# IN2-ViAUn/Exploration-of-Potential

Hardware: AMD Instinct MI355X
Metric: training images/sec, YOLOX-l 24p 640x640 bf16 (higher is better)
Workload: dtype bf16; 1 GPU; YOLOX-l-24p (CSPDarknet53+PAFPN+24p head) train step, 640x640, batch 20/GPU, 10 GTs/img, SimOTA + 24-circle GIoU loss, SGD nesterov; global_batch=20, parallelism=dp1, hip_graph=forward and backward as two lanes of captured segments, loss, update

## Files before the change

exploration-of-potential_amd/csrc/elementwise.hip:

```cpp
#include <stdio.h>
#include <stdlib.h>
#include "common.h"

namespace {

constexpr int MAX_BLOCKS = 2048;

__device__ __forceinline__ void load8(const bf16* p, float (&v)[8]) {
    bf16x8 t = *reinterpret_cast<const bf16x8*>(p);
#pragma unroll
    for (int i = 0; i < 8; ++i) v[i] = (float)t[i];
}
__device__ __forceinline__ void store8(bf16* p, const float (&v)[8]) {
    bf16x8 t;
#pragma unroll
    for (int i = 0; i < 8; ++i) t[i] = (bf16)v[i];
    *reinterpret_cast<bf16x8*>(p) = t;
}

__device__ __forceinline__ long pinned_row(long m) {
    asm volatile("" : "+v"(m));
    return m;
}

// ... 481 lines not shown
            const int yy = py + dy;
            if (yy < 0 || yy >= H) continue;
            for (int dx = -6; dx <= 6; ++dx) {
                const int xx = px + dx;
                if (xx < 0 || xx >= W) continue;
                float v[8];
                load8(x + ((long)(n * H + yy) * W + xx) * ld_x + cg * 8, v);
                const uint8_t code = (uint8_t)(((dy + 8) << 4) | (dx + 8));
                const bool in9 = dy >= -4 && dy <= 4 && dx >= -4 && dx <= 4;
                const bool in5 = dy >= -2 && dy <= 2 && dx >= -2 && dx <= 2;
#pragma unroll
                for (int j = 0; j < 8; ++j) {
                    if (v[j] > m13[j] || v[j] != v[j]) { m13[j] = v[j]; i13[j] = code; }
                    if (in9 && (v[j] > m9[j] || v[j] != v[j])) { m9[j] = v[j]; i9[j] = code; }
                    if (in5 && (v[j] > m5[j] || v[j] != v[j])) { m5[j] = v[j]; i5[j] = code; }
                }
            }
        }
        store8(y5 + pix * ld_y + cg * 8, m5);
        store8(y9 + pix * ld_y + cg * 8, m9);
        store8(y13 + pix * ld_y + cg * 8, m13);
        uint8_t* ip = idx + pix * C + cg * 8;
#pragma unroll
        for (int j = 0; j < 8; ++j) { ip[j] = i5[j]; ip[plane + j] = i9[j]; ip[2 * plane + j] = i13[j]; }
    }
}

__global__ __launch_bounds__(256) void spp_row_kernel(const bf16* x, long ld_x, bf16* h, uint8_t* hx, int B, int H, int W, int C) {
    const int cgs = C >> 3;
    const long total = (long)B * H * W * cgs;
    const long plane = (long)B * H * W * C;
    for (long i = (long)blockIdx.x * 256 + threadIdx.x; i < total; i += (long)gridDim.x * 256) {
        const int cg = (int)(i % cgs);
        const long pix = i / cgs;
        const int px = (int)(pix % W);
        float m5[8], m9[8], m13[8];
        uint8_t i5[8], i9[8], i13[8];
#pragma unroll
        for (int j = 0; j < 8; ++j) { m5[j] = m9[j] = m13[j] = -INFINITY; i5[j] = i9[j] = i13[j] = 8; }
#pragma unroll
        for (int dx = -6; dx <= 6; ++dx) {
            const int xx = px + dx;
            if (xx < 0 || xx >= W) continue;
            float v[8];
            load8(x + (pix + dx) * ld_x + cg * 8, v);
            const uint8_t code = (uint8_t)(dx + 8);
            const bool in9 = dx >= -4 && dx <= 4, in5 = dx >= -2 && dx <= 2;
#pragma unroll
            for (int j = 0; j < 8; ++j) {
                if (v[j] > m13[j] || v[j] != v[j]) { m13[j] = v[j]; i13[j] = code; }
                if (in9 && (v[j] > m9[j] || v[j] != v[j])) { m9[j] = v[j]; i9[j] = code; }
                if (in5 && (v[j] > m5[j] || v[j] != v[j])) { m5[j] = v[j]; i5[j] = code; }
            }
        }
        bf16* hp = h + pix * C + cg * 8;
        store8(hp, m5); store8(hp + plane, m9); store8(hp + 2 * plane, m13);
        uint8_t* ip = hx + pix * C + cg * 8;
#pragma unroll
        for (int j = 0; j < 8; ++j) { ip[j] = i5[j]; ip[plane + j] = i9[j]; ip[2 * plane + j] = i13[j]; }
    }
}

__global__ __launch_bounds__(256) void spp_col_kernel(const bf16* h, const uint8_t* hx, bf16* y5, bf16* y9, bf16* y13, long ld_y,
                                                      uint8_t* idx, int B, int H, int W, int C) {
    const int cgs = C >> 3;
    const long total = (long)B * H * W * cgs;
    const long plane = (long)B * H * W * C;
    for (long i = (long)blockIdx.x * 256 + threadIdx.x; i < total; i += (long)gridDim.x * 256) {
        const int cg = (int)(i % cgs);
        const long pix = i / cgs;
        const int py = (int)((pix / W) % H);
        float m[3][8];
        uint8_t id[3][8];
#pragma unroll
        for (int w = 0; w < 3; ++w)
#pragma unroll
            for (int j = 0; j < 8; ++j) { m[w][j] = -INFINITY; id[w][j] = 0x88; }
#pragma unroll
        for (int dy = -6; dy <= 6; ++dy) {
            const int yy = py + dy;
            if (yy < 0 || yy >= H) continue;
            const long q = (pix + (long)dy * W) * C + cg * 8;
#pragma unroll
            for (int w = 0; w < 3; ++w) {
                const int r = 2 + 2 * w;
                if (dy < -r || dy > r) continue;
                float v[8];
                load8(h + w * plane + q, v);
                const uint2 cx = *reinterpret_cast<const uint2*>(hx + w * plane + q);
#pragma unroll
                for (int j = 0; j < 8; ++j) {
                    const unsigned c = ((j < 4 ? cx.x : cx.y) >> (8 * (j & 3))) & 0xFF;
                    if (v[j] > m[w][j] || v[j] != v[j]) { m[w][j] = v[j]; id[w][j] = (uint8_t)(((dy + 8) << 4) | c); }
                }
            }
        }
        store8(y5 + pix * ld_y + cg * 8, m[0]);
        store8(y9 + pix * ld_y + cg * 8, m[1]);
        store8(y13 + pix * ld_y + cg * 8, m[2]);
        uint8_t* ip = idx + pix * C + cg * 8;
#pragma unroll
        for (int j = 0; j < 8; ++j) { ip[j] = id[0][j]; ip[plane + j] = id[1][j]; ip[2 * plane + j] = id[2][j]; }
    }
}

__global__ __launch_bounds__(256) void spp_bwd_kernel(const bf16* dy5, const bf16* dy9, const bf16* dy13, long ld_dy,
                                                      const uint8_t* idx, bf16* dx, long ld_dx, int accumulate, int B,
                                                      int H, int W, int C) {
    const int cgs = C >> 3;
    const long total = (long)B * H * W * cgs;
    const long plane = (long)B * H * W * C;
    for (long i = (long)blockIdx.x * 256 + threadIdx.x; i < total; i += (long)gridDim.x * 256) {
        const int cg = (int)(i % cgs);
        const long pix = i / cgs;
        const int n = (int)(pix / (H * W));
        const int rem = (int)(pix - (long)n * H * W);
        const int py = rem / W, px = rem - py * W;
        float acc[8] = {0, 0, 0, 0, 0, 0, 0, 0};
        for (int dy = -6; dy <= 6; ++dy) {
            const int oy = py - dy;
            if (oy < 0 || oy >= H) continue;
            for (int dxo = -6; dxo <= 6; ++dxo) {
                const int ox = px - dxo;
                if (ox < 0 || ox >= W) continue;
                const long op = (long)(n * H + oy) * W + ox;
                const uint8_t code = (uint8_t)(((dy + 8) << 4) | (dxo + 8));
                const uint8_t* ip = idx + op * C + cg * 8;
                const unsigned rep = code * 0x01010101u;
                auto gather = [&](const bf16* g, const uint8_t* codes) {
                    uint2 c = *reinterpret_cast<const uint2*>(codes);
                    c.x ^= rep; c.y ^= rep;
                    float v[8];
                    load8(g + op * ld_dy + cg * 8, v);
#pragma unroll
                    for (int j = 0; j < 8; ++j)
                        if ((((j < 4 ? c.x : c.y) >> (8 * (j & 3))) & 0xFFu) == 0u) acc[j] += v[j];
                };
                gather(dy13, ip + 2 * plane);
                if (dy >= -4 && dy <= 4 && dxo >= -4 && dxo <= 4) gather(dy9, ip + plane);
                if (dy >= -2 && dy <= 2 && dxo >= -2 && dxo <= 2) gather(dy5, ip);
            }
        }
        bf16* d = dx + pix * ld_dx + cg * 8;
        if (accumulate) {
            float o[8];
            load8(d, o);
#pragma unroll
            for (int j = 0; j < 8; ++j) acc[j] += o[j];
        }
        store8(d, acc);
    }
}

__global__ __launch_bounds__(256) void spp_bwd_lds_kernel(const bf16* dy5, const bf16* dy9, const bf16* dy13, long ld_dy,
                                                          const uint8_t* idx, bf16* dx, long ld_dx, int accumulate, int B,
                                                          int H, int W, int C) {
    extern __shared__ __attribute__((aligned(16))) char spp_lds[];
    const int HW = H * W;
    bf16x8* gv = reinterpret_cast<bf16x8*>(spp_lds);
    uint2* cv = reinterpret_cast<uint2*>(spp_lds + (size_t)3 * HW * 16);
    float* gh = reinterpret_cast<float*>(spp_lds + (size_t)3 * HW * 24);
    uint2* ds = reinterpret_cast<uint2*>(spp_lds + (size_t)3 * HW * 24 + (size_t)HW * 32);
    const int cg = blockIdx.x, n = blockIdx.y;
    const long plane = (long)B * HW * C;
    const long base = (long)n * HW;
    for (int q = threadIdx.x; q < HW; q += 256) {
        const long op = base + q;
        gv[q] = *reinterpret_cast<const bf16x8*>(dy5 + op * ld_dy + cg * 8);
        gv[HW + q] = *reinterpret_cast<const bf16x8*>(dy9 + op * ld_dy + cg * 8);
        gv[2 * HW + q] = *reinterpret_cast<const bf16x8*>(dy13 + op * ld_dy + cg * 8);
        const uint8_t* ip = idx + op * C + cg * 8;
        cv[q] = *reinterpret_cast<const uint2*>(ip);
        cv[HW + q] = *reinterpret_cast<const uint2*>(ip + plane);
        cv[2 * HW + q] = *reinterpret_cast<const uint2*>(ip + 2 * plane);
    }
    __syncthreads();
    constexpr int NPASS = 4;
    float acc[NPASS][8];
#pragma unroll
    for (int t = 0; t < NPASS; ++t)
#pragma unroll
        for (int j = 0; j < 8; ++j) acc[t][j] = 0.f;
    for (int pool = 2; pool >= 0; --pool) {
        const int R = 2 * pool + 2;
        for (int q = threadIdx.x; q < HW; q += 256) {
            const int r = q / W, x = q - r * W;
            float s[8] = {0, 0, 0, 0, 0, 0, 0, 0};
            unsigned char sel[8];
#pragma unroll
            for (int j = 0; j < 8; ++j) sel[j] = 0xFF;
            for (int dy = -R; dy <= R; ++dy) {
                const int y = r - dy;
                if (y < 0 || y >= H) continue;
                const int o = y * W + x;
                const uint2 c = cv[pool * HW + o];
                const bf16x8 t = gv[pool * HW + o];
#pragma unroll
                for (int j = 0; j < 8; ++j) {
                    const unsigned byte = ((j < 4 ? c.x : c.y) >> (8 * (j & 3))) & 0xFFu;
                    if ((int)(byte >> 4) == dy + 8) { s[j] += (float)t[j]; sel[j] = (unsigned char)(byte & 15u); }
                }
            }
#pragma unroll
            for (int j = 0; j < 8; ++j) gh[q * 8 + j] = s[j];
            uint2 d;
            d.x = sel[0] | (sel[1] << 8) | (sel[2] << 16) | ((unsigned)sel[3] << 24);
            d.y = sel[4] | (sel[5] << 8) | (sel[6] << 16) | ((unsigned)sel[7] << 24);
            ds[q] = d;
        }
        __syncthreads();
#pragma unroll
        for (int t = 0; t < NPASS; ++t) {
            const int q = threadIdx.x + 256 * t;
            if (q < HW) {
                const int r = q / W, c = q - r * W;
                for (int dxo = -R; dxo <= R; ++dxo) {
                    const int x = c - dxo;
                    if (x < 0 || x >= W) continue;
                    const int o = r * W + x;
                    const uint2 d = ds[o];
#pragma unroll
                    for (int j = 0; j < 8; ++j) {
                        const unsigned byte = ((j < 4 ? d.x : d.y) >> (8 * (j & 3))) & 0xFFu;
                        if ((int)byte == dxo + 8) acc[t][j] += gh[o * 8 + j];
                    }
                }
            }
        }
        __syncthreads();
    }
#pragma unroll
    for (int t = 0; t < NPASS; ++t) {
        const int q = threadIdx.x + 256 * t;
        if (q < HW) {
            bf16* d = dx + (base + q) * ld_dx + cg * 8;
            float out[8];
#pragma unroll
            for (int j = 0; j < 8; ++j) out[j] = acc[t][j];
            if (accumulate) {
                float o[8];
                load8(d, o);
#pragma unroll
                for (int j = 0; j < 8; ++j) out[j] += o[j];
            }
            store8(d, out);
        }
    }
}

__global__ __launch_bounds__(256) void upsample2_fwd_kernel(const bf16* x, long ld_x, bf16* y, long ld_y, int B, int H,
                                                            int W, int C) {
    const int cgs = C >> 3;
    const long total = (long)B * 2 * H * 2 * W * cgs;
    for (long i = (long)blockIdx.x * 256 + threadIdx.x; i < total; i += (long)gridDim.x * 256) {
        const int cg = (int)(i % cgs);
        const long opix = i / cgs;
        const int n = (int)(opix / (4 * H * W));
        const int rem = (int)(opix - (long)n * 4 * H * W);
        const int oy = rem / (2 * W), ox = rem - oy * 2 * W;
        const long ip = (long)(n * H + (oy >> 1)) * W + (ox >> 1);
        *reinterpret_cast<bf16x8*>(y + opix * ld_y + cg * 8) = *reinterpret_cast<const bf16x8*>(x + ip * ld_x + cg * 8);
    }
}

__global__ __launch_bounds__(256) void upsample2_bwd_kernel(const bf16* dy, long ld_dy, bf16* dx, long ld_dx,
                                                            int accumulate, int B, int H, int W, int C) {
    const int cgs = C >> 3;
    const long total = (long)B * H * W * cgs;
    for (long i = (long)blockIdx.x * 256 + threadIdx.x; i < total; i += (long)gridDim.x * 256) {
        const int cg = (int)(i % cgs);
        const long pix = i / cgs;
        const int n = (int)(pix / (H * W));
        const int rem = (int)(pix - (long)n * H * W);
        const int py = rem / W, px = rem - py * W;
        float acc[8] = {0, 0, 0, 0, 0, 0, 0, 0};
#pragma unroll
        for (int a = 0; a < 2; ++a)
#pragma unroll
            for (int b = 0; b < 2; ++b) {
                float v[8];
                load8(dy + ((long)(n * 2 * H + 2 * py + a) * 2 * W + 2 * px + b) * ld_dy + cg * 8, v);
#pragma unroll
                for (int j = 0; j < 8; ++j) acc[j] += v[j];
            }
        bf16* d = dx + pix * ld_dx + cg * 8;
        if (accumulate) {
            float o[8];
            load8(d, o);
#pragma unroll
            for (int j = 0; j < 8; ++j) acc[j] += o[j];
        }
        store8(d, acc);
    }
}

__global__ __launch_bounds__(256) void rows_copy_kernel(const bf16* src, long ld_src, bf16* dst, long ld_dst,
                                                        int accumulate, long M, int C) {
    const int cgs = C >> 3;
    const long total = M * cgs;
    for (long i = (long)blockIdx.x * 256 + threadIdx.x; i < total; i += (long)gridDim.x * 256) {
        const int cg = (int)(i % cgs);
        const long m = i / cgs;
        bf16* d = dst + m * ld_dst + cg * 8;
        if (!accumulate) {
            *reinterpret_cast<bf16x8*>(d) = *reinterpret_cast<const bf16x8*>(src + m * ld_src + cg * 8);
            continue;
        }
        float v[8], o[8];
        load8(src + m * ld_src + cg * 8, v);
        load8(d, o);
#pragma unroll
        for (int j = 0; j < 8; ++j) v[j] += o[j];
        store8(d, v);
    }
}

__global__ __launch_bounds__(256) void cast_f32_bf16_kernel(const float* src, bf16* dst, long n4) {
    for (long i = (long)blockIdx.x * 256 + threadIdx.x; i < n4; i += (long)gridDim.x * 256) {
        const float4 v = reinterpret_cast<const float4*>(src)[i];
        bf16x4 o = {(bf16)v.x, (bf16)v.y, (bf16)v.z, (bf16)v.w};
        reinterpret_cast<bf16x4*>(dst)[i] = o;
    }
}
__global__ __launch_bounds__(256) void cast_bf16_f32_kernel(const bf16* src, float* dst, long n4) {
    for (long i = (long)blockIdx.x * 256 + threadIdx.x; i < n4; i += (long)gridDim.x * 256) {
        const bf16x4 v = reinterpret_cast<const bf16x4*>(src)[i];
        reinterpret_cast<float4*>(dst)[i] = make_float4((float)v[0], (float)v[1], (float)v[2], (float)v[3]);
    }
}

__global__ __launch_bounds__(256) void decode_fwd_kernel(float* out, int B, int A, int a0, int H, int W, float s,
                                                         int ncols, float* origin) {
    const long total = (long)B * H * W * 26;
    for (long i = (long)blockIdx.x * 256 + threadIdx.x; i < total; i += (long)gridDim.x * 256) {
        const int c = (int)(i % 26);
        const long cell = i / 26;
        const int n = (int)(cell / (H * W));
        const int hw = (int)(cell - (long)n * H * W);
        float* p = out + ((long)n * A + a0 + hw) * ncols + c;
        const float t = *p;
        if (origin) origin[((long)n * A + a0 + hw) * 26 + c] = t;
        float v;
        if (c == 0) v = (t + (float)(hw % W)) * s;
        else if (c == 1) v = (t + (float)(hw / W)) * s;
        else v = expf(t) * s;
        *p = v;
    }
}

__global__ __launch_bounds__(256) void decode_bwd_kernel(const float* dout, const float* out, bf16* d_regobj, bf16* d_cls,
                                                         int B, int A, int a0, int H, int W, float s, int ncols,
                                                         const float* d_origin) {
    const int C = ncols - 27;
    const int ld_cls = (C + 7) & ~7;
    const int chunks = 4 + (ld_cls >> 3);
    const long total = (long)B * H * W * chunks;
    for (long i = (long)blockIdx.x * 256 + threadIdx.x; i < total; i += (long)gridDim.x * 256) {
        const int chunk = (int)(i % chunks);
        const long cell = i / chunks;
        const int n = (int)(cell / (H * W));
        const int hw = (int)(cell - (long)n * H * W);
        const long row = ((long)n * A + a0 + hw) * ncols;
        bf16x8 o;
        if (chunk < 4) {
#pragma unroll
            for (int j = 0; j < 8; ++j) {
                const int c = chunk * 8 + j;
                float g = 0.f;
                if (c < 2) g = dout[row + c] * s;
                else if (c < 26) g = dout[row + c] * out[row + c];
                else if (c == 26) g = dout[row + 26];
                if (d_origin && c < 26) g += d_origin[((long)n * A + a0 + hw) * 26 + c];
                o[j] = (bf16)g;
            }
            *reinterpret_cast<bf16x8*>(d_regobj + cell * 32 + chunk * 8) = o;
        } else {
            const int k = chunk - 4;
#pragma unroll
            for (int j = 0; j < 8; ++j) {
                const int c = k * 8 + j;
                o[j] = (bf16)(c < C ? dout[row + 27 + c] : 0.f);
            }
            *reinterpret_cast<bf16x8*>(d_cls + cell * ld_cls + k * 8) = o;
        }
    }
}

__global__ __launch_bounds__(256) void colsum_kernel(const bf16* g, long ld, float* db, long M, int N) {
    __shared__ float red[256];
    for (int c0 = 0; c0 < N; c0 += 64) {
        const int c = c0 + (threadIdx.x & 63);
// ... 233 lines not shown
            for (long k = i; k < n; ++k) {
                float gg = g[k] * gscale;
                if (DECAY) gg = decay_grp[(base + k) >> 6] != 0 ? gg + decay * p[k] : gg;
                const float b = first ? gg : mom * buf[k] + gg;
                buf[k] = b;
                p[k] -= lr * (gg + mom * b);
                if (ema) ema[k] = ema_step(ema[k], p[k], d, omd);
                const int wd = wf_delta ? wf_delta[(base + k) >> 6] : WF_NONE;
                if (wd != WF_NONE) wf[base + k + wd] = (bf16)p[k];
            }
        }
    }
}

__global__ __launch_bounds__(256) void ema_kernel(float* ema, const float* src, long n, float d, float omd, const float* hp) {
    if (hp) { d = hp[3]; omd = hp[4]; }
    for (long i = (long)blockIdx.x * 256 + threadIdx.x; i < n; i += (long)gridDim.x * 256) ema[i] = ema_step(ema[i], src[i], d, omd);
}

__global__ void set_hparams_kernel(float* hp, float lr, float mom, float gscale, float d, float omd) {
    hp[0] = lr; hp[1] = mom; hp[2] = gscale; hp[3] = d; hp[4] = omd;
}
__global__ void set_hparams_decay_kernel(float* hp, float lr, float mom, float gscale, float d, float omd, float decay) {
    hp[0] = lr; hp[1] = mom; hp[2] = gscale; hp[3] = d; hp[4] = omd; hp[5] = decay;
}
__global__ void clear_flag_kernel(int* f) { *f = 0; }

int cap_grid(long work_items) {
    long b = (work_items + 255) / 256;
    return (int)(b < 1 ? 1 : (b > MAX_BLOCKS ? MAX_BLOCKS : b));
}

}

#define S_ (hipStream_t) stream

extern "C" int ep24_bn_act_fwd(const void* z, int64_t ld_z, const int64_t* stats, int reps, const float* gamma,
                               const float* beta, float* running_mean, float* running_var, int64_t* num_batches,
                               int64_t* num_batches2, float* save, void* y, int64_t ld_y, const void* residual, int64_t ld_res,
                               int64_t M, int C, float eps, float momentum, int act, void* stream) {
    EP24_REQUIRE(act >= 0 && act <= 3, EP24_E_ARG, "bn_act_fwd: act=%d is none of 0 identity, 1 SiLU, 2 ReLU, 3 LeakyReLU(0.1)", act);
    EP24_REQUIRE(z && stats && gamma && beta && save && y, EP24_E_ARG, "bn_act_fwd: null pointer");
    EP24_REQUIRE(C % 8 == 0 && ld_z % 8 == 0 && ld_y % 8 == 0 && (!residual || ld_res % 8 == 0), EP24_E_ARG,
                 "bn_act_fwd: C=%d / strides must be multiples of 8", C);
    EP24_REQUIRE(M > 0 && reps > 0, EP24_E_ARG, "bn_act_fwd: empty");
    const int fw_per = (C >= 1024 || (C <= 128 && M * C >= (12L << 20))) ? 8 : 4;
    const int grid = flat_grid(M, C, fw_per);
    const bool fixed = (grid * 256L) % (C >> 3) == 0;
    auto kfn = fixed ? fwd_kernel<true>(act, residual != nullptr) : fwd_kernel<false>(act, residual != nullptr);
    hipLaunchKernelGGL(kfn, dim3(grid), dim3(256), 2 * (C + C / 8) * sizeof(float), S_, (const bf16*)z, ld_z, (const long long*)stats, reps, gamma,
                       beta, running_mean, running_var, (long*)num_batches, (long*)num_batches2, save, (bf16*)y, ld_y, (const bf16*)residual,
                       ld_res, M, C, eps, momentum);
    EP24_LAUNCH_CHECK("ep24_bn_act_fwd");
    return EP24_OK;
}

extern "C" int ep24_bn_act_bwd_reduce(const void* dy, int64_t ld_dy, const void* z, int64_t ld_z, const float* save,
                                      const float* gamma, const float* beta, int64_t* dgamma, int64_t* dbeta, int64_t M, int C,
                                      int act, int reps, void* stream) {
    EP24_REQUIRE(act >= 0 && act <= 3, EP24_E_ARG, "bn_act_bwd_reduce: act=%d is none of 0 identity, 1 SiLU, 2 ReLU, 3 LeakyReLU(0.1)", act);
    EP24_REQUIRE(dy && z && save && gamma && beta && dgamma && dbeta && reps > 0, EP24_E_ARG, "bn_act_bwd_reduce: null pointer / reps");
    EP24_REQUIRE(C % 8 == 0 && ld_dy % 8 == 0 && ld_z % 8 == 0, EP24_E_ARG, "bn_act_bwd_reduce: alignment");
    int red_cap = 512;
    int red_rows = 4;
    auto kfn = act == 1 ? bn_act_bwd_reduce_kernel<4, 256, 1> : act == 2 ? bn_act_bwd_reduce_kernel<4, 256, 2> : act == 3 ? bn_act_bwd_reduce_kernel<4, 256, 3> : bn_act_bwd_reduce_kernel<4, 256, 0>;
    hipLaunchKernelGGL(kfn, dim3(rows_grid(M, C, red_rows, red_cap, 256)), dim3(256), 0, S_, (const bf16*)dy, ld_dy, (const bf16*)z, ld_z,
                       save, gamma, beta, (long long*)dgamma, (long long*)dbeta, M, C, reps);
    EP24_LAUNCH_CHECK("ep24_bn_act_bwd_reduce");
    return EP24_OK;
}

extern "C" int ep24_bn_act_bwd_apply(const void* dy, int64_t ld_dy, const void* z, int64_t ld_z, const float* save,
                                     const float* gamma, const float* beta, const int64_t* dgamma, const int64_t* dbeta,
                                     float* gamma_grad, float* beta_grad, void* dz, int64_t ld_dz, int64_t M, int C, int act,
                                     int reps, void* stream) {
    EP24_REQUIRE(act >= 0 && act <= 3, EP24_E_ARG, "bn_act_bwd_apply: act=%d is none of 0 identity, 1 SiLU, 2 ReLU, 3 LeakyReLU(0.1)", act);
    EP24_REQUIRE(dy && z && save && gamma && beta && dgamma && dbeta && dz && reps > 0, EP24_E_ARG, "bn_act_bwd_apply: null pointer / reps");
    EP24_REQUIRE(C % 8 == 0 && ld_dy % 8 == 0 && ld_z % 8 == 0 && ld_dz % 8 == 0, EP24_E_ARG, "bn_act_bwd_apply: alignment");
    EP24_REQUIRE((((uintptr_t)save | (uintptr_t)gamma | (uintptr_t)beta) & 15) == 0, EP24_E_ARG,
                 "bn_act_bwd_apply: save / gamma / beta must be 16-byte aligned (they are read as vectors)");
    EP24_REQUIRE((((uintptr_t)gamma_grad | (uintptr_t)beta_grad) & 15) == 0, EP24_E_ARG, "bn_act_bwd_apply: gamma_grad / beta_grad must be 16-byte aligned");
    const int ap_rows = M * C <= (16L << 20) ? 8 : 16, ap_cap = 2048;
    auto kfn = act == 1 ? bn_act_bwd_apply_kernel<4, 1> : act == 2 ? bn_act_bwd_apply_kernel<4, 2> : act == 3 ? bn_act_bwd_apply_kernel<4, 3> : bn_act_bwd_apply_kernel<4, 0>;
    hipLaunchKernelGGL(kfn, dim3(rows_grid(M, C, ap_rows, ap_cap)), dim3(256), 2 * (size_t)C * sizeof(float), S_, (const bf16*)dy, ld_dy,
                       (const bf16*)z, ld_z, save, gamma, beta, (const long long*)dgamma, (const long long*)dbeta, gamma_grad, beta_grad,
                       (bf16*)dz, ld_dz, M, C, reps);
    EP24_LAUNCH_CHECK("ep24_bn_act_bwd_apply");
    return EP24_OK;
}

extern "C" int ep24_bn_act_bwd_fused(const void* dy, int64_t ld_dy, const void* z, int64_t ld_z, const float* save, const float* gamma,
                                     const float* beta, int64_t* dgamma, int64_t* dbeta, float* gamma_grad, float* beta_grad, void* dz,
                                     int64_t ld_dz, int64_t M, int C, int act, int reps, int32_t* barrier, void* stream) {
    EP24_REQUIRE(act >= 0 && act <= 3, EP24_E_ARG, "bn_act_bwd_fused: act=%d is none of 0 identity, 1 SiLU, 2 ReLU, 3 LeakyReLU(0.1)", act);
    EP24_REQUIRE(dy && z && save && gamma && beta && dgamma && dbeta && dz && barrier && reps > 0, EP24_E_ARG, "bn_act_bwd_fused: null pointer / reps");
    EP24_REQUIRE(C % 8 == 0 && C <= 2048 && ld_dy % 8 == 0 && ld_z % 8 == 0 && ld_dz % 8 == 0, EP24_E_ARG, "bn_act_bwd_fused: alignment / C <= 2048");
    EP24_REQUIRE((((uintptr_t)save | (uintptr_t)gamma | (uintptr_t)beta | (uintptr_t)gamma_grad | (uintptr_t)beta_grad) & 15) == 0, EP24_E_ARG,
                 "bn_act_bwd_fused: save / gamma / beta and their gradients must be 16-byte aligned (they are read as vectors)");
    int grid = rows_grid(M, C, 4, 256, 256);
    auto kfn = act == 1 ? bn_act_bwd_fused_kernel<1> : act == 2 ? bn_act_bwd_fused_kernel<2> : act == 3 ? bn_act_bwd_fused_kernel<3> : bn_act_bwd_fused_kernel<0>;
    hipLaunchKernelGGL(kfn, dim3(grid), dim3(256), 2 * (size_t)C * sizeof(float), S_, (const bf16*)dy, ld_dy, (const bf16*)z, ld_z, save, gamma, beta,
                       (long long*)dgamma, (long long*)dbeta, gamma_grad, beta_grad, (bf16*)dz, ld_dz, M, C, reps, (unsigned*)barrier);
    EP24_LAUNCH_CHECK("ep24_bn_act_bwd_fused");
    return EP24_OK;
}

namespace ep24_igemm {
int bn_barrier_timeouts() {
    unsigned v = 0;
    if (hipMemcpyFromSymbol(&v, HIP_SYMBOL(g_bn_barrier_timeouts), sizeof(v)) != hipSuccess) return -1;
    return (int)v;
}
}

extern "C" int ep24_bn_act_bwd_apply_acc(const void* dy, int64_t ld_dy, const void* z, int64_t ld_z, const float* save,
                                         const float* gamma, const float* beta, const int64_t* dgamma, const int64_t* dbeta,
                                         float* gamma_grad, float* beta_grad, void* dz, int64_t ld_dz, int64_t M, int C, int act,
                                         int reps, void* stream) {
    EP24_REQUIRE(act >= 0 && act <= 3, EP24_E_ARG, "bn_act_bwd_apply_acc: act=%d is none of 0 identity, 1 SiLU, 2 ReLU, 3 LeakyReLU(0.1)", act);
    EP24_REQUIRE(dy && z && save && gamma && beta && dgamma && dbeta && dz && reps > 0, EP24_E_ARG, "bn_act_bwd_apply_acc: null pointer / reps");
    EP24_REQUIRE(C % 8 == 0 && ld_dy % 8 == 0 && ld_z % 8 == 0 && ld_dz % 8 == 0, EP24_E_ARG, "bn_act_bwd_apply_acc: alignment");
    EP24_REQUIRE((((uintptr_t)save | (uintptr_t)gamma | (uintptr_t)beta) & 15) == 0, EP24_E_ARG,
                 "bn_act_bwd_apply_acc: save / gamma / beta must be 16-byte aligned (they are read as vectors)");
    EP24_REQUIRE((((uintptr_t)gamma_grad | (uintptr_t)beta_grad) & 15) == 0, EP24_E_ARG, "bn_act_bwd_apply_acc: gamma_grad / beta_grad must be 16-byte aligned");
    auto kfn = act == 1 ? bn_act_bwd_apply_kernel<4, 1, true> : act == 2 ? bn_act_bwd_apply_kernel<4, 2, true> : act == 3 ? bn_act_bwd_apply_kernel<4, 3, true> : bn_act_bwd_apply_kernel<4, 0, true>;
    hipLaunchKernelGGL(kfn, dim3(rows_grid(M, C, 16, 2048)), dim3(256), 2 * (size_t)C * sizeof(float), S_, (const bf16*)dy, ld_dy, (const bf16*)z, ld_z, save, gamma, beta,
                       (const long long*)dgamma, (const long long*)dbeta, gamma_grad, beta_grad, (bf16*)dz, ld_dz, M, C, reps);
    EP24_LAUNCH_CHECK("ep24_bn_act_bwd_apply_acc");
    return EP24_OK;
}

extern "C" int ep24_stem_pack(const float* images, void* rows, int64_t ld, int B, int H, int W, void* stream) {
    EP24_REQUIRE(images && rows && H % 2 == 0 && W % 2 == 0 && B > 0 && ld >= 108 && ld % 8 == 0, EP24_E_ARG, "stem_pack: bad arguments");
    EP24_REQUIRE(((uintptr_t)images & 7) == 0, EP24_E_ARG, "stem_pack: images must be 8-byte aligned (the kernel loads pixel pairs)");
    long sp_blocks = ((long)B * (H / 2) * (W / 2) + 31) / 32;
    hipLaunchKernelGGL(stem_pack_kernel, dim3((unsigned)(sp_blocks > 16384 ? 16384 : sp_blocks)), dim3(256), 0, S_, images,
                       (bf16*)rows, B, H, W, (int)ld);
    EP24_LAUNCH_CHECK("ep24_stem_pack");
    return EP24_OK;
}

extern "C" int ep24_focus_pack(const float* images, void* f16, int B, int H, int W, void* stream) {
    EP24_REQUIRE(images && f16 && H % 2 == 0 && W % 2 == 0 && B > 0 && (reinterpret_cast<unsigned long long>(images) & 7) == 0, EP24_E_ARG,
                 "focus_pack: bad arguments");
    const long blocks = ((long)B * (H / 2) * (W / 2) + 255) / 256;
    hipLaunchKernelGGL(focus_pack_kernel, dim3((unsigned)(blocks > 65536 ? 65536 : blocks)), dim3(256), 0, S_, images, (bf16*)f16, B, H, W);
    EP24_LAUNCH_CHECK("ep24_focus_pack");
    return EP24_OK;
}

extern "C" int ep24_spp_fwd(const void* x, int64_t ld_x, void* y5, void* y9, void* y13, int64_t ld_y, uint8_t* idx, int B,
                            int H, int W, int C, void* scratch, void* stream) {
    EP24_REQUIRE(x && y5 && y9 && y13 && idx && C % 8 == 0 && ld_x % 8 == 0 && ld_y % 8 == 0, EP24_E_ARG, "spp_fwd: bad arguments");
    if (scratch) {
        const long n = (long)B * H * W * C;
        EP24_REQUIRE(((uintptr_t)scratch & 7) == 0, EP24_E_ARG, "spp_fwd: scratch must be 8-byte aligned");
        bf16* h = (bf16*)scratch;
        uint8_t* hx = (uint8_t*)scratch + 6 * n;
        hipLaunchKernelGGL(spp_row_kernel, dim3(cap_grid(n / 8)), dim3(256), 0, S_, (const bf16*)x, ld_x, h, hx, B, H, W, C);
        hipLaunchKernelGGL(spp_col_kernel, dim3(cap_grid(n / 8)), dim3(256), 0, S_, (const bf16*)h, (const uint8_t*)hx, (bf16*)y5,
                           (bf16*)y9, (bf16*)y13, ld_y, idx, B, H, W, C);
        EP24_LAUNCH_CHECK("ep24_spp_fwd");
        return EP24_OK;
    }
    hipLaunchKernelGGL(spp_fwd_kernel, dim3(cap_grid((long)B * H * W * (C / 8))), dim3(256), 0, S_, (const bf16*)x, ld_x,
                       (bf16*)y5, (bf16*)y9, (bf16*)y13, ld_y, idx, B, H, W, C);
    EP24_LAUNCH_CHECK("ep24_spp_fwd");
    return EP24_OK;
}

extern "C" int ep24_spp_bwd(const void* dy5, const void* dy9, const void* dy13, int64_t ld_dy, const uint8_t* idx, void* dx,
                            int64_t ld_dx, int accumulate, int B, int H, int W, int C, void* stream) {
    EP24_REQUIRE(dy5 && dy9 && dy13 && idx && dx && C % 8 == 0 && ld_dy % 8 == 0 && ld_dx % 8 == 0, EP24_E_ARG, "spp_bwd: bad arguments");
    EP24_REQUIRE(((uintptr_t)idx & 7) == 0, EP24_E_ARG, "spp_bwd: idx must be 8-byte aligned (8 winner codes per load)");
    const size_t lds = (size_t)H * W * 112;
    if (lds <= 64 * 1024 && H * W <= 1024)
        hipLaunchKernelGGL(spp_bwd_lds_kernel, dim3(C / 8, B), dim3(256), lds, S_, (const bf16*)dy5, (const bf16*)dy9, (const bf16*)dy13,
                           ld_dy, idx, (bf16*)dx, ld_dx, accumulate, B, H, W, C);
    else
        hipLaunchKernelGGL(spp_bwd_kernel, dim3(cap_grid((long)B * H * W * (C / 8))), dim3(256), 0, S_, (const bf16*)dy5,
                           (const bf16*)dy9, (const bf16*)dy13, ld_dy, idx, (bf16*)dx, ld_dx, accumulate, B, H, W, C);
    EP24_LAUNCH_CHECK("ep24_spp_bwd");
    return EP24_OK;
}

extern "C" int ep24_upsample2_fwd(const void* x, int64_t ld_x, void* y, int64_t ld_y, int B, int H, int W, int C, void* stream) {
    EP24_REQUIRE(x && y && C % 8 == 0 && ld_x % 8 == 0 && ld_y % 8 == 0, EP24_E_ARG, "upsample2_fwd: bad arguments");
    hipLaunchKernelGGL(upsample2_fwd_kernel, dim3(cap_grid((long)B * 4 * H * W * (C / 8))), dim3(256), 0, S_, (const bf16*)x,
                       ld_x, (bf16*)y, ld_y, B, H, W, C);
    EP24_LAUNCH_CHECK("ep24_upsample2_fwd");
    return EP24_OK;
}

extern "C" int ep24_upsample2_bwd(const void* dy, int64_t ld_dy, void* dx, int64_t ld_dx, int accumulate, int B, int H, int W,
                                  int C, void* stream) {
    EP24_REQUIRE(dy && dx && C % 8 == 0 && ld_dy % 8 == 0 && ld_dx % 8 == 0, EP24_E_ARG, "upsample2_bwd: bad arguments");
    hipLaunchKernelGGL(upsample2_bwd_kernel, dim3(cap_grid((long)B * H * W * (C / 8))), dim3(256), 0, S_, (const bf16*)dy, ld_dy,
                       (bf16*)dx, ld_dx, accumulate, B, H, W, C);
    EP24_LAUNCH_CHECK("ep24_upsample2_bwd");
    return EP24_OK;
}

extern "C" int ep24_rows_copy(const void* src, int64_t ld_src, void* dst, int64_t ld_dst, int accumulate, int64_t M, int C,
                              void* stream) {
    EP24_REQUIRE(src && dst && C % 8 == 0 && ld_src % 8 == 0 && ld_dst % 8 == 0, EP24_E_ARG, "rows_copy: bad arguments");
    hipLaunchKernelGGL(rows_copy_kernel, dim3(cap_grid(M * (C / 8))), dim3(256), 0, S_, (const bf16*)src, ld_src, (bf16*)dst,
                       ld_dst, accumulate, M, C);
    EP24_LAUNCH_CHECK("ep24_rows_copy");
    return EP24_OK;
}

extern "C" int ep24_cast_f32_bf16(const float* src, void* dst, int64_t n, void* stream) {
    EP24_REQUIRE(src && dst && n % 4 == 0 && n >= 0, EP24_E_ARG, "cast_f32_bf16: n must be a multiple of 4");
    EP24_REQUIRE((uintptr_t)src % 16 == 0 && (uintptr_t)dst % 8 == 0, EP24_E_ARG, "cast_f32_bf16: src must be 16-byte, dst 8-byte aligned");
    if (n) hipLaunchKernelGGL(cast_f32_bf16_kernel, dim3(cap_grid(n / 4)), dim3(256), 0, S_, src, (bf16*)dst, (long)(n / 4));
    EP24_LAUNCH_CHECK("ep24_cast_f32_bf16");
    return EP24_OK;
}

extern "C" int ep24_cast_bf16_f32(const void* src, float* dst, int64_t n, void* stream) {
    EP24_REQUIRE(src && dst && n % 4 == 0 && n >= 0, EP24_E_ARG, "cast_bf16_f32: n must be a multiple of 4");
    EP24_REQUIRE((uintptr_t)src % 8 == 0 && (uintptr_t)dst % 16 == 0, EP24_E_ARG, "cast_bf16_f32: src must be 8-byte, dst 16-byte aligned");
    if (n) hipLaunchKernelGGL(cast_bf16_f32_kernel, dim3(cap_grid(n / 4)), dim3(256), 0, S_, (const bf16*)src, dst, (long)(n / 4));
    EP24_LAUNCH_CHECK("ep24_cast_bf16_f32");
    return EP24_OK;
}

extern "C" int ep24_head_decode_fwd(float* out, int B, int A, int a0, int H, int W, float stride, int ncols, float* origin,
                                    void* stream) {
    EP24_REQUIRE(out && a0 >= 0 && a0 + H * W <= A && ncols >= 27, EP24_E_ARG, "head_decode_fwd: bad arguments");
    hipLaunchKernelGGL(decode_fwd_kernel, dim3(cap_grid((long)B * H * W * 26)), dim3(256), 0, S_, out, B, A, a0, H, W, stride, ncols, origin);
    EP24_LAUNCH_CHECK("ep24_head_decode_fwd");
    return EP24_OK;
}

extern "C" int ep24_head_decode_bwd(const float* dout, const float* out, void* d_regobj, void* d_cls, int B, int A, int a0,
                                    int H, int W, float stride, int ncols, const float* d_origin, void* stream) {
    EP24_REQUIRE(dout && out && d_regobj && d_cls && a0 >= 0 && a0 + H * W <= A && ncols > 27, EP24_E_ARG,
                 "head_decode_bwd: bad arguments");
    hipLaunchKernelGGL(decode_bwd_kernel, dim3(cap_grid((long)B * H * W * (4 + (ncols - 27 + 7) / 8))), dim3(256), 0, S_, dout, out, (bf16*)d_regobj,
                       (bf16*)d_cls, B, A, a0, H, W, stride, ncols, d_origin);
    EP24_LAUNCH_CHECK("ep24_head_decode_bwd");
    return EP24_OK;
}

extern "C" int ep24_colsum_splits(int64_t M) {
    long blocks = (M + 3) / 4;
    return (int)(blocks > 64 ? 64 : (blocks < 1 ? 1 : blocks));
}

extern "C" int ep24_colsum_slab(const void* g, int64_t ld, float* slab, int64_t M, int N, void* stream) {
    EP24_REQUIRE(g && slab && N > 0 && N <= 2048 && M > 0 && ld % 8 == 0 && ld >= ((N + 7) / 8) * 8, EP24_E_ARG,
                 "colsum_slab: bad arguments (rows must be padded to a multiple of 8 columns)");
    hipLaunchKernelGGL(colsum_slab_kernel, dim3((unsigned)ep24_colsum_splits(M)), dim3(256), 0, S_, (const bf16*)g, ld, slab, M, N);
    EP24_LAUNCH_CHECK("ep24_colsum_slab");
    return EP24_OK;
}

extern "C" int ep24_colsum(const void* g, int64_t ld, float* db, int64_t M, int N, void* stream) {
    EP24_REQUIRE(g && db && N > 0, EP24_E_ARG, "colsum: bad arguments");
    long blocks = (M + 3) / 4;
    if (blocks > 512) blocks = 512;
    hipLaunchKernelGGL(colsum_kernel, dim3((unsigned)blocks), dim3(256), 0, S_, (const bf16*)g, ld, db, M, N);
    EP24_LAUNCH_CHECK("ep24_colsum");
    return EP24_OK;
}

extern "C" int ep24_pack_weights(const float* w, int64_t ld_w, void* w_fwd, void* w_dgrad, int Cout, int T, int Cin, int Cin_pad,
                                 int Cout_pad, void* stream) {
    EP24_REQUIRE(w && (w_fwd || w_dgrad) && Cin_pad >= Cin && Cout_pad >= Cout, EP24_E_ARG, "pack_weights: bad arguments");
    long n = (long)Cout * T * Cin;
    hipLaunchKernelGGL(pack_weights_kernel, dim3(cap_grid(n)), dim3(256), 0, S_, w, ld_w, (bf16*)w_fwd, (bf16*)w_dgrad, Cout, T, Cin,
                       Cin_pad, Cout_pad);
    EP24_LAUNCH_CHECK("ep24_pack_weights");
    return EP24_OK;
}

extern "C" int ep24_sgd_nesterov(float* p, const float* g, float* buf, int64_t n, float lr, float momentum, float grad_scale,
                                 int32_t* first_flag, void* stream) {
    EP24_REQUIRE(p && g && buf && first_flag && n > 0, EP24_E_ARG, "sgd_nesterov: bad arguments");
    EP24_REQUIRE(((uintptr_t)p | (uintptr_t)g | (uintptr_t)buf) % 16 == 0, EP24_E_ARG, "sgd_nesterov: 16-byte alignment");
    hipLaunchKernelGGL(sgd_kernel<false>, dim3(cap_grid((n + 3) / 4)), dim3(256), 0, S_, p, g, buf, n, lr, momentum, grad_scale, first_flag,
                       (const float*)nullptr, (float*)nullptr, 0L, (const int*)nullptr, (bf16*)nullptr);
    hipLaunchKernelGGL(clear_flag_kernel, dim3(1), dim3(1), 0, S_, first_flag);
    EP24_LAUNCH_CHECK("ep24_sgd_nesterov");
    return EP24_OK;
}

extern "C" int ep24_sgd_nesterov_hp(float* p, const float* g, float* buf, int64_t n, const float* hp, int32_t* first_flag,
                                    float* ema, void* stream) {
    EP24_REQUIRE(p && g && buf && hp && first_flag && n > 0, EP24_E_ARG, "sgd_nesterov_hp: bad arguments");
    EP24_REQUIRE(((uintptr_t)p | (uintptr_t)g | (uintptr_t)buf | (uintptr_t)ema) % 16 == 0, EP24_E_ARG, "sgd_nesterov_hp: 16-byte alignment");
    hipLaunchKernelGGL(sgd_kernel<false>, dim3(cap_grid((n + 3) / 4)), dim3(256), 0, S_, p, g, buf, n, 0.f, 0.f, 0.f, first_flag, hp, ema,
                       0L, (const int*)nullptr, (bf16*)nullptr);
    hipLaunchKernelGGL(clear_flag_kernel, dim3(1), dim3(1), 0, S_, first_flag);
    EP24_LAUNCH_CHECK("ep24_sgd_nesterov_hp");
    return EP24_OK;
}

extern "C" int ep24_sgd_nesterov_hp_range(float* p, const float* g, float* buf, int64_t first, int64_t n, const float* hp,
                                          int32_t* first_flag, float* ema, int last, void* stream) {
    EP24_REQUIRE(p && g && buf && hp && first_flag && n > 0 && first >= 0 && first % 4 == 0, EP24_E_ARG, "sgd_nesterov_hp_range: bad arguments");
    EP24_REQUIRE(((uintptr_t)p | (uintptr_t)g | (uintptr_t)buf | (uintptr_t)ema) % 16 == 0, EP24_E_ARG, "sgd_nesterov_hp_range: 16-byte alignment");
    hipLaunchKernelGGL(sgd_kernel<false>, dim3(cap_grid((n + 3) / 4)), dim3(256), 0, S_, p + first, g + first, buf + first, n, 0.f, 0.f, 0.f, first_flag, hp,
                       ema ? ema + first : nullptr, 0L, (const int*)nullptr, (bf16*)nullptr);
    if (last) hipLaunchKernelGGL(clear_flag_kernel, dim3(1), dim3(1), 0, S_, first_flag);
    EP24_LAUNCH_CHECK("ep24_sgd_nesterov_hp_range");
    return EP24_OK;
}

extern "C" int ep24_sgd_nesterov_hp_range_pack(float* p, const float* g, float* buf, int64_t first, int64_t n, const float* hp,
                                               int32_t* first_flag, float* ema, int last, const int32_t* wf_delta, void* wf, void* stream) {
    EP24_REQUIRE(p && g && buf && hp && first_flag && wf_delta && wf && n > 0 && first >= 0 && first % 4 == 0, EP24_E_ARG,
                 "sgd_nesterov_hp_range_pack: bad arguments");
    EP24_REQUIRE(((uintptr_t)p | (uintptr_t)g | (uintptr_t)buf | (uintptr_t)ema) % 16 == 0 && (uintptr_t)wf % 16 == 0, EP24_E_ARG,
                 "sgd_nesterov_hp_range_pack: 16-byte alignment");
    hipLaunchKernelGGL(sgd_kernel<false>, dim3(cap_grid((n + 3) / 4)), dim3(256), 0, S_, p + first, g + first, buf + first, n, 0.f, 0.f, 0.f, first_flag, hp,
                       ema ? ema + first : nullptr, (long)first, (const int*)wf_delta, (bf16*)wf);
    if (last) hipLaunchKernelGGL(clear_flag_kernel, dim3(1), dim3(1), 0, S_, first_flag);
    EP24_LAUNCH_CHECK("ep24_sgd_nesterov_hp_range_pack");
    return EP24_OK;
}

extern "C" int ep24_sgd_nesterov_decay(float* p, const float* g, float* buf, int64_t n, float lr, float momentum, float grad_scale,
                                       float weight_decay, const uint8_t* decay_grp, int32_t* first_flag, void* stream) {
    EP24_REQUIRE(p && g && buf && decay_grp && first_flag && n > 0, EP24_E_ARG, "sgd_nesterov_decay: bad arguments");
    EP24_REQUIRE(((uintptr_t)p | (uintptr_t)g | (uintptr_t)buf) % 16 == 0, EP24_E_ARG, "sgd_nesterov_decay: 16-byte alignment");
    hipLaunchKernelGGL((sgd_kernel<true, float, const uint8_t*>), dim3(cap_grid((n + 3) / 4)), dim3(256), 0, S_, p, g, buf, n, lr, momentum,
                       grad_scale, first_flag, (const float*)nullptr, (float*)nullptr, 0L, (const int*)nullptr, (bf16*)nullptr, weight_decay, decay_grp);
    hipLaunchKernelGGL(clear_flag_kernel, dim3(1), dim3(1), 0, S_, first_flag);
    EP24_LAUNCH_CHECK("ep24_sgd_nesterov_decay");
// ... 88 lines not shown
```

Baseline: 1023 images/s.

## Fuse SPP max-pool forward into LDS cascade and scatter-based backward

Adds a forward SPP kernel that keeps one channel-group image plane in shared memory and computes the 5/9/13 max pools as a cascade of separable 5-wide windows. It packs a sortable value key and position into each word so an unsigned max also yields the winner index. The backward pass is rewritten from a per-output gather over window offsets into a two-stage scatter (column then row) into padded LDS accumulators, and prefetches the next pool's gradients. Block order is swizzled across channel groups. This removes the intermediate row/col scratch passes and the wide gather loops, at the cost of more complex tie and NaN encoding and more shared memory per block.

```diff
diff --git a/exploration-of-potential_amd/csrc/elementwise.hip b/exploration-of-potential_amd/csrc/elementwise.hip
--- a/exploration-of-potential_amd/csrc/elementwise.hip
+++ b/exploration-of-potential_amd/csrc/elementwise.hip
@@ -657,91 +657,252 @@
     }
 }
 
-__global__ __launch_bounds__(256) void spp_bwd_lds_kernel(const bf16* dy5, const bf16* dy9, const bf16* dy13, long ld_dy,
-                                                          const uint8_t* idx, bf16* dx, long ld_dx, int accumulate, int B,
-                                                          int H, int W, int C) {
+constexpr int SPP_LDS_RULE_BYTES = 112;
+
+__device__ __forceinline__ int spp_group(int b, int cgs) { return (cgs & 7) ? b : (b & 7) * (cgs >> 3) + (b >> 3); }
+
+struct SppE { uint4 lo, hi; };
+
+__device__ __forceinline__ unsigned spp_leaf(unsigned b, unsigned pos) {
+    const unsigned key = b ^ ((b & 0x8000u) ? 0xFFFFu : 0x8000u);
+    unsigned w = (key << 16) | ((0x3FFFu - pos) << 2);
+    if (b == 0x8000u) w = (0x8000u << 16) | ((0x3FFFu - pos) << 2) | 1u;
+    if (b == 0xFF80u) w = 0x007F0000u;
+    if ((b & 0x7FFFu) > 0x7F80u) w = 0xFFFF0000u | (pos << 2);
+    return w;
+}
+__device__ __forceinline__ unsigned spp_pick(unsigned L, unsigned R) { return L > R ? L : R; }
+__device__ __forceinline__ SppE spp_comb(const SppE& L, const SppE& R) {
+    SppE o;
+    o.lo = make_uint4(spp_pick(L.lo.x, R.lo.x), spp_pick(L.lo.y, R.lo.y), spp_pick(L.lo.z, R.lo.z), spp_pick(L.lo.w, R.lo.w));
+    o.hi = make_uint4(spp_pick(L.hi.x, R.hi.x), spp_pick(L.hi.y, R.hi.y), spp_pick(L.hi.z, R.hi.z), spp_pick(L.hi.w, R.hi.w));
+    return o;
+}
+__device__ __forceinline__ SppE spp_ld(const uint4* pl, int HW, int q) { return {pl[q], pl[HW + q]}; }
+__device__ __forceinline__ void spp_st(uint4* pl, int HW, int q, const SppE& e) { pl[q] = e.lo; pl[HW + q] = e.hi; }
+__device__ __forceinline__ int spp_clamp(int v, int n) { return v < 0 ? 0 : (v >= n ? n - 1 : v); }
+__device__ __forceinline__ SppE spp_w5(const uint4* pl, int HW, int q0, int stride, int p, int n) {
+    SppE a = spp_ld(pl, HW, q0 + spp_clamp(p - 2, n) * stride);
+#pragma unroll
+    for (int d = -1; d <= 2; ++d) a = spp_comb(a, spp_ld(pl, HW, q0 + spp_clamp(p + d, n) * stride));
+    return a;
+}
+__device__ __forceinline__ SppE spp_pair(const uint4* pl, int HW, int q0, int stride, int p, int n) {
+    return spp_comb(spp_ld(pl, HW, q0 + spp_clamp(p - 2, n) * stride), spp_ld(pl, HW, q0 + spp_clamp(p + 2, n) * stride));
+}
+__device__ __forceinline__ unsigned spp_unpack(unsigned w, unsigned here) {
+    const unsigned key = w >> 16;
+    const unsigned b = (key ^ ((key & 0x8000u) ? 0x8000u : 0xFFFFu)) | ((w & 1u) << 15);
+    const unsigned f = (w >> 2) & 0x3FFFu;
+    const unsigned t = (key == 0xFFFFu ? f : 0x3FFFu - f) + 0x408u - here;
+    const unsigned code = key == 0x007Fu ? 0x88u : (((t >> 3) & 0xF0u) | (t & 0xFu));
+    return b | (code << 16);
+}
+__device__ __forceinline__ void spp_emit(const SppE& e, int y, int x, bf16* yp, uint8_t* ip) {
+    const unsigned here = ((unsigned)y << 7) | (unsigned)x;
+    const unsigned u[8] = {spp_unpack(e.lo.x, here), spp_unpack(e.lo.y, here), spp_unpack(e.lo.z, here), spp_unpack(e.lo.w, here),
+                           spp_unpack(e.hi.x, here), spp_unpack(e.hi.y, here), spp_unpack(e.hi.z, here), spp_unpack(e.hi.w, here)};
+    uint4 v;
+    v.x = (u[0] & 0xFFFFu) | (u[1] << 16);
+    v.y = (u[2] & 0xFFFFu) | (u[3] << 16);
+    v.z = (u[4] & 0xFFFFu) | (u[5] << 16);
+    v.w = (u[6] & 0xFFFFu) | (u[7] << 16);
+    *reinterpret_cast<uint4*>(yp) = v;
+    uint2 c;
+    c.x = (u[0] >> 16) | ((u[1] >> 16) << 8) | ((u[2] >> 16) << 16) | ((u[3] >> 16) << 24);
+    c.y = (u[4] >> 16) | ((u[5] >> 16) << 8) | ((u[6] >> 16) << 16) | ((u[7] >> 16) << 24);
+    *reinterpret_cast<uint2*>(ip) = c;
+}
+
+__global__ __launch_bounds__(512) void spp_fwd_lds_kernel(const bf16* x, long ld_x, bf16* y5, bf16* y9, bf16* y13, long ld_y,
+                                                          uint8_t* idx, int B, int H, int W, int C) {
     extern __shared__ __attribute__((aligned(16))) char spp_lds[];
     const int HW = H * W;
-    bf16x8* gv = reinterpret_cast<bf16x8*>(spp_lds);
-    uint2* cv = reinterpret_cast<uint2*>(spp_lds + (size_t)3 * HW * 16);
-    float* gh = reinterpret_cast<float*>(spp_lds + (size_t)3 * HW * 24);
-    uint2* ds = reinterpret_cast<uint2*>(spp_lds + (size_t)3 * HW * 24 + (size_t)HW * 32);
-    const int cg = blockIdx.x, n = blockIdx.y;
+    uint4* PA = reinterpret_cast<uint4*>(spp_lds);
+    uint4* PB = PA + 2 * HW;
+    uint4* PC = PB + 2 * HW;
+    const int cg = spp_group(blockIdx.x, gridDim.x), n = blockIdx.y;
     const long plane = (long)B * HW * C;
     const long base = (long)n * HW;
-    for (int q = threadIdx.x; q < HW; q += 256) {
-        const long op = base + q;
-        gv[q] = *reinterpret_cast<const bf16x8*>(dy5 + op * ld_dy + cg * 8);
-        gv[HW + q] = *reinterpret_cast<const bf16x8*>(dy9 + op * ld_dy + cg * 8);
-        gv[2 * HW + q] = *reinterpret_cast<const bf16x8*>(dy13 + op * ld_dy + cg * 8);
-        const uint8_t* ip = idx + op * C + cg * 8;
-        cv[q] = *reinterpret_cast<const uint2*>(ip);
-        cv[HW + q] = *reinterpret_cast<const uint2*>(ip + plane);
-        cv[2 * HW + q] = *reinterpret_cast<const uint2*>(ip + 2 * plane);
-    }
+    int q[2], py[2], px[2];
+    uint4 raw[2];
+#pragma unroll
+    for (int k = 0; k < 2; ++k) {
+        q[k] = threadIdx.x + k * blockDim.x;
+        py[k] = q[k] / W;
+        px[k] = q[k] - py[k] * W;
+        if (q[k] < HW) raw[k] = *reinterpret_cast<const uint4*>(x + (base + q[k]) * ld_x + cg * 8);
+    }
+#pragma unroll
+    for (int k = 0; k < 2; ++k)
+        if (q[k] < HW) {
+            const unsigned d[4] = {raw[k].x, raw[k].y, raw[k].z, raw[k].w};
+            const unsigned pos = ((unsigned)py[k] << 7) | (unsigned)px[k];
+            unsigned w[8];
+#pragma unroll
+            for (int j = 0; j < 8; ++j) w[j] = spp_leaf((j & 1) ? (d[j >> 1] >> 16) : (d[j >> 1] & 0xFFFFu), pos);
+            spp_st(PA, HW, q[k], {make_uint4(w[0], w[1], w[2], w[3]), make_uint4(w[4], w[5], w[6], w[7])});
+        }
     __syncthreads();
-    constexpr int NPASS = 4;
-    float acc[NPASS][8];
-#pragma unroll
-    for (int t = 0; t < NPASS; ++t)
-#pragma unroll
-        for (int j = 0; j < 8; ++j) acc[t][j] = 0.f;
+#pragma unroll
+    for (int k = 0; k < 2; ++k)
+        if (q[k] < HW) spp_st(PB, HW, q[k], spp_w5(PA, HW, py[k] * W, 1, px[k], W));
+    __syncthreads();
+    bf16* o5 = y5 + cg * 8;
+    bf16* o9 = y9 + cg * 8;
+    bf16* o13 = y13 + cg * 8;
+    uint8_t* oi = idx + cg * 8;
+#pragma unroll
+    for (int k = 0; k < 2; ++k)
+        if (q[k] < HW) {
+            spp_st(PA, HW, q[k], spp_pair(PB, HW, py[k] * W, 1, px[k], W));
+            spp_emit(spp_w5(PB, HW, px[k], W, py[k], H), py[k], px[k], o5 + (base + q[k]) * ld_y, oi + (base + q[k]) * C);
+        }
+    __syncthreads();
+#pragma unroll
+    for (int k = 0; k < 2; ++k)
+        if (q[k] < HW) {
+            spp_st(PB, HW, q[k], spp_pair(PA, HW, py[k] * W, 1, px[k], W));
+            spp_st(PC, HW, q[k], spp_w5(PA, HW, px[k], W, py[k], H));
+        }
+    __syncthreads();
+#pragma unroll
+    for (int k = 0; k < 2; ++k)
+        if (q[k] < HW) {
+            spp_emit(spp_pair(PC, HW, px[k], W, py[k], H), py[k], px[k], o9 + (base + q[k]) * ld_y, oi + plane + (base + q[k]) * C);
+            spp_st(PA, HW, q[k], spp_w5(PB, HW, px[k], W, py[k], H));
+        }
+    __syncthreads();
+#pragma unroll
+    for (int k = 0; k < 2; ++k)
+        if (q[k] < HW) spp_st(PB, HW, q[k], spp_pair(PA, HW, px[k], W, py[k], H));
+    __syncthreads();
+#pragma unroll
+    for (int k = 0; k < 2; ++k)
+        if (q[k] < HW)
+            spp_emit(spp_pair(PB, HW, px[k], W, py[k], H), py[k], px[k], o13 + (base + q[k]) * ld_y, oi + 2 * plane + (base + q[k]) * C);
+}
+
+__device__ __forceinline__ void spp_add4(float* plane, const int (&a)[4], const float (&g)[4]) {
+    float p0 = plane[a[0]], p1 = plane[a[1]], p2 = plane[a[2]], p3 = plane[a[3]];
+    asm volatile("" : "+v"(p0), "+v"(p1), "+v"(p2), "+v"(p3));
+    const float v0 = p0 + g[0];
+    const float v1 = (a[1] == a[0] ? v0 : p1) + g[1];
+    const float v2 = (a[2] == a[1] ? v1 : a[2] == a[0] ? v0 : p2) + g[2];
+    const float v3 = (a[3] == a[2] ? v2 : a[3] == a[1] ? v1 : a[3] == a[0] ? v0 : p3) + g[3];
+    plane[a[0]] = v0;
+    plane[a[1]] = v1;
+    plane[a[2]] = v2;
+    plane[a[3]] = v3;
+}
+
+__global__ __launch_bounds__(256) void spp_bwd_scatter_kernel(const bf16* dy5, const bf16* dy9, const bf16* dy13, long ld_dy,
+                                                              const uint8_t* idx, bf16* dx, long ld_dx, int accumulate, int B,
+                                                              int H, int W, int C, int Wp) {
+    extern __shared__ __attribute__((aligned(16))) char spp_lds[];
+    const int HW = H * W, HWp = H * Wp;
+    float* Gs = reinterpret_cast<float*>(spp_lds);
+    float* dX = Gs + (size_t)HWp * 8;
+    bf16x8* gv = reinterpret_cast<bf16x8*>(dX + (size_t)HWp * 8);
+    uint64_t* cv = reinterpret_cast<uint64_t*>(gv + HW);
+    uint8_t* sel = reinterpret_cast<uint8_t*>(cv + HW);
+    const unsigned short* gs = reinterpret_cast<const unsigned short*>(gv);
+    const uint8_t* cs = reinterpret_cast<const uint8_t*>(cv);
+    const int cg = spp_group(blockIdx.x, gridDim.x), n = blockIdx.y;
+    const long plane = (long)B * HW * C;
+    const long base = (long)n * HW;
+    constexpr int NPASS = 3;
+    bf16x8 pg[NPASS];
+    uint64_t pc[NPASS];
+    auto fetch = [&](int pool) {
+        const bf16* g = (pool == 2 ? dy13 : pool == 1 ? dy9 : dy5) + cg * 8;
+        const uint8_t* ip = idx + pool * plane + cg * 8;
+#pragma unroll
+        for (int k = 0; k < NPASS; ++k) {
+            const int q = min((int)threadIdx.x + 256 * k, HW - 1);
+            pg[k] = *reinterpret_cast<const bf16x8*>(g + (base + q) * ld_dy);
+            pc[k] = *reinterpret_cast<const uint64_t*>(ip + (base + q) * C);
+        }
+    };
+    auto stage = [&]() {
+#pragma unroll
+        for (int k = 0; k < NPASS; ++k) {
+            const int q = threadIdx.x + 256 * k;
+            if (q < HW) { gv[q] = pg[k]; cv[q] = pc[k]; }
+        }
+        for (int i = threadIdx.x; i < HWp * 2; i += 256) reinterpret_cast<float4*>(Gs)[i] = make_float4(0.f, 0.f, 0.f, 0.f);
+        for (int i = threadIdx.x; i < HWp; i += 256) reinterpret_cast<uint2*>(sel)[i] = make_uint2(0xFFFFFFFFu, 0xFFFFFFFFu);
+    };
+    fetch(2);
+    for (int i = threadIdx.x; i < HWp * 2; i += 256) reinterpret_cast<float4*>(dX)[i] = make_float4(0.f, 0.f, 0.f, 0.f);
+    stage();
+    __syncthreads();
+#pragma unroll
     for (int pool = 2; pool >= 0; --pool) {
-        const int R = 2 * pool + 2;
-        for (int q = threadIdx.x; q < HW; q += 256) {
+        if (pool > 0) fetch(pool - 1);
+        for (int t = threadIdx.x; t < W * 8; t += 256) {
+            const int x = t >> 3, ch = t & 7;
+            for (int y0 = 0; y0 < H; y0 += 4) {
+                unsigned c[4];
+                float g[4];
+#pragma unroll
+                for (int u = 0; u < 4; ++u) {
+                    const int o = (min(y0 + u, H - 1) * W + x) * 8 + ch;
+                    c[u] = cs[o];
+                    g[u] = __uint_as_float((unsigned)gs[o] << 16);
+                }
+                int a[4];
+                bool ok[4];
+#pragma unroll
+                for (int u = 0; u < 4; ++u) {
+                    const int r = y0 + u + (int)(c[u] >> 4) - 8;
+                    ok[u] = y0 + u < H && (unsigned)r < (unsigned)H;
+                    a[u] = ((ok[u] ? r : min(y0 + u, H - 1)) * Wp + x) * 8 + ch;
+                    g[u] = ok[u] ? g[u] : 0.f;
+                }
+                spp_add4(Gs, a, g);
+#pragma unroll
+                for (int u = 0; u < 4; ++u)
+                    if (ok[u]) sel[a[u]] = (uint8_t)(c[u] & 15u);
+            }
+        }
+        __syncthreads();
+        for (int t = threadIdx.x; t < H * 8; t += 256) {
+            const int r = t >> 3, ch = t & 7;
+            for (int x0 = 0; x0 < W; x0 += 4) {
+                unsigned s[4];
+                float g[4];
+#pragma unroll
+                for (int u = 0; u < 4; ++u) {
+                    const int o = (r * Wp + min(x0 + u, W - 1)) * 8 + ch;
+                    s[u] = sel[o];
+                    g[u] = Gs[o];
+                }
+                int a[4];
+#pragma unroll
+                for (int u = 0; u < 4; ++u) {
+                    const int xt = x0 + u + (int)s[u] - 8;
+                    const bool ok = x0 + u < W && s[u] != 0xFFu && (unsigned)xt < (unsigned)W;
+                    a[u] = (r * Wp + (ok ? xt : min(x0 + u, W - 1))) * 8 + ch;
+                    g[u] = ok ? g[u] : 0.f;
+                }
+                spp_add4(dX, a, g);
+            }
+        }
+        __syncthreads();
+        if (pool > 0) {
+            stage();
+            __syncthreads();
+        }
+    }
+#pragma unroll
+    for (int k = 0; k < NPASS; ++k) {
+        const int q = threadIdx.x + 256 * k;
+        if (q < HW) {
             const int r = q / W, x = q - r * W;
-            float s[8] = {0, 0, 0, 0, 0, 0, 0, 0};
-            unsigned char sel[8];
-#pragma unroll
-            for (int j = 0; j < 8; ++j) sel[j] = 0xFF;
-            for (int dy = -R; dy <= R; ++dy) {
-                const int y = r - dy;
-                if (y < 0 || y >= H) continue;
-                const int o = y * W + x;
-                const uint2 c = cv[pool * HW + o];
-                const bf16x8 t = gv[pool * HW + o];
-#pragma unroll
-                for (int j = 0; j < 8; ++j) {
-                    const unsigned byte = ((j < 4 ? c.x : c.y) >> (8 * (j & 3))) & 0xFFu;
-                    if ((int)(byte >> 4) == dy + 8) { s[j] += (float)t[j]; sel[j] = (unsigned char)(byte & 15u); }
-                }
-            }
-#pragma unroll
-            for (int j = 0; j < 8; ++j) gh[q * 8 + j] = s[j];
-            uint2 d;
-            d.x = sel[0] | (sel[1] << 8) | (sel[2] << 16) | ((unsigned)sel[3] << 24);
-            d.y = sel[4] | (sel[5] << 8) | (sel[6] << 16) | ((unsigned)sel[7] << 24);
-            ds[q] = d;
-        }
-        __syncthreads();
-#pragma unroll
-        for (int t = 0; t < NPASS; ++t) {
-            const int q = threadIdx.x + 256 * t;
-            if (q < HW) {
-                const int r = q / W, c = q - r * W;
-                for (int dxo = -R; dxo <= R; ++dxo) {
-                    const int x = c - dxo;
-                    if (x < 0 || x >= W) continue;
-                    const int o = r * W + x;
-                    const uint2 d = ds[o];
-#pragma unroll
-                    for (int j = 0; j < 8; ++j) {
-                        const unsigned byte = ((j < 4 ? d.x : d.y) >> (8 * (j & 3))) & 0xFFu;
-                        if ((int)byte == dxo + 8) acc[t][j] += gh[o * 8 + j];
-                    }
-                }
-            }
-        }
-        __syncthreads();
-    }
-#pragma unroll
-    for (int t = 0; t < NPASS; ++t) {
-        const int q = threadIdx.x + 256 * t;
-        if (q < HW) {
+            const float4 a = reinterpret_cast<const float4*>(dX)[(r * Wp + x) * 2], b = reinterpret_cast<const float4*>(dX)[(r * Wp + x) * 2 + 1];
+            float out[8] = {a.x, a.y, a.z, a.w, b.x, b.y, b.z, b.w};
             bf16* d = dx + (base + q) * ld_dx + cg * 8;
-            float out[8];
-#pragma unroll
-            for (int j = 0; j < 8; ++j) out[j] = acc[t][j];
             if (accumulate) {
                 float o[8];
                 load8(d, o);
@@ -1281,9 +1442,17 @@
 extern "C" int ep24_spp_fwd(const void* x, int64_t ld_x, void* y5, void* y9, void* y13, int64_t ld_y, uint8_t* idx, int B,
                             int H, int W, int C, void* scratch, void* stream) {
     EP24_REQUIRE(x && y5 && y9 && y13 && idx && C % 8 == 0 && ld_x % 8 == 0 && ld_y % 8 == 0, EP24_E_ARG, "spp_fwd: bad arguments");
+    EP24_REQUIRE(((uintptr_t)scratch & 7) == 0, EP24_E_ARG, "spp_fwd: scratch must be 8-byte aligned");
+    if ((size_t)H * W * SPP_LDS_RULE_BYTES <= 64 * 1024 && H > 0 && W > 0 && H <= 127 && W <= 127 && B > 0 && B <= 65535 && C > 0 &&
+        ((uintptr_t)idx & 7) == 0) {
+        const int hw = H * W, threads = hw >= 512 ? 512 : (hw + 63) / 64 * 64;
+        hipLaunchKernelGGL(spp_fwd_lds_kernel, dim3(C / 8, B), dim3(threads), (size_t)hw * 96, S_, (const bf16*)x, ld_x, (bf16*)y5,
+                           (bf16*)y9, (bf16*)y13, ld_y, idx, B, H, W, C);
+        EP24_LAUNCH_CHECK("ep24_spp_fwd");
+        return EP24_OK;
+    }
     if (scratch) {
         const long n = (long)B * H * W * C;
-        EP24_REQUIRE(((uintptr_t)scratch & 7) == 0, EP24_E_ARG, "spp_fwd: scratch must be 8-byte aligned");
         bf16* h = (bf16*)scratch;
         uint8_t* hx = (uint8_t*)scratch + 6 * n;
         hipLaunchKernelGGL(spp_row_kernel, dim3(cap_grid(n / 8)), dim3(256), 0, S_, (const bf16*)x, ld_x, h, hx, B, H, W, C);
@@ -1302,10 +1471,13 @@
                             int64_t ld_dx, int accumulate, int B, int H, int W, int C, void* stream) {
     EP24_REQUIRE(dy5 && dy9 && dy13 && idx && dx && C % 8 == 0 && ld_dy % 8 == 0 && ld_dx % 8 == 0, EP24_E_ARG, "spp_bwd: bad arguments");
     EP24_REQUIRE(((uintptr_t)idx & 7) == 0, EP24_E_ARG, "spp_bwd: idx must be 8-byte aligned (8 winner codes per load)");
-    const size_t lds = (size_t)H * W * 112;
-    if (lds <= 64 * 1024 && H * W <= 1024)
-        hipLaunchKernelGGL(spp_bwd_lds_kernel, dim3(C / 8, B), dim3(256), lds, S_, (const bf16*)dy5, (const bf16*)dy9, (const bf16*)dy13,
-                           ld_dy, idx, (bf16*)dx, ld_dx, accumulate, B, H, W, C);
+    if ((size_t)H * W * SPP_LDS_RULE_BYTES <= 64 * 1024 && H > 0 && W > 0 && B > 0 && B <= 65535 && C > 0) {
+        int Wp = W | 1;
+        size_t lds = (size_t)H * W * 24 + (size_t)H * Wp * 72;
+        if (lds > 64 * 1024) { Wp = W; lds = (size_t)H * W * 96; }
+        hipLaunchKernelGGL(spp_bwd_scatter_kernel, dim3(C / 8, B), dim3(256), lds, S_, (const bf16*)dy5, (const bf16*)dy9, (const bf16*)dy13,
+                           ld_dy, idx, (bf16*)dx, ld_dx, accumulate, B, H, W, C, Wp);
+    }
     else
         hipLaunchKernelGGL(spp_bwd_kernel, dim3(cap_grid((long)B * H * W * (C / 8))), dim3(256), 0, S_, (const bf16*)dy5,
                            (const bf16*)dy9, (const bf16*)dy13, ld_dy, idx, (bf16*)dx, ld_dx, accumulate, B, H, W, C);
```

Measured after the change: 1031 images/s (median of 6 runs). No clear change (+0.8%).
